# catniplab/vlgp

Hardware: AMD Instinct MI355X
Metric: EM iterations/sec (higher is better)
Workload: dtype f64

## Files before the change

### include/vlgp_hip.h

```cpp
#ifndef VLGP_HIP_H
#define VLGP_HIP_H

#include <stdint.h>

#ifdef __cplusplus
extern "C" {
#endif

#define VLGP_ABI_VERSION 3
#define VLGP_MAX_SETS 4
#define VLGP_MAX_L 64
#define VLGP_MAX_XDIM 64
#define VLGP_MAX_RANK 64
#define VLGP_UNIQUE_ID_BYTES 128

#define VLGP_OK 0
#define VLGP_ERR_ARG (-1)
#define VLGP_ERR_HIP (-2)
#define VLGP_ERR_STATE (-3)
#define VLGP_ERR_COMM (-4)

typedef struct vlgp_ctx vlgp_ctx;

int vlgp_abi_version(void);
// ... 138 lines not shown
#define VLGP_PATH_HSTEP_GENERIC 4
#define VLGP_PATH_HSTEP_OLD 5
#define VLGP_PATH_HSTEP_MIXED 6
int vlgp_debug_last_hstep_path(vlgp_ctx* ctx, int* path);
int vlgp_debug_reload_switches(vlgp_ctx* ctx);
int vlgp_debug_switch(vlgp_ctx* ctx, const char* name, double* value);
int vlgp_debug_live_memory(int64_t out[4]);
int vlgp_debug_hstep_stats(vlgp_ctx* ctx, double out[4]);
#define VLGP_HP_PATH 0
#define VLGP_HP_TC 1
#define VLGP_HP_N_LR 2
#define VLGP_HP_N_ROUGH 3
#define VLGP_HP_RMAX 4
#define VLGP_HP_CLASS 5
#define VLGP_HP_TABG 6
#define VLGP_HP_FUSED 7
#define VLGP_HP_NB 8
#define VLGP_HP_LDS 9
#define VLGP_HP_WLM 10
#define VLGP_HP_NW 11
#define VLGP_HP_TM_GLOBAL 12
#define VLGP_HP_HUGE 13
#define VLGP_HP_RERUN 14
#define VLGP_HP_RCAP 15
#define VLGP_HSTEP_PLAN_LEN 31
int vlgp_debug_hstep_plan(vlgp_ctx* ctx, int out[VLGP_HSTEP_PLAN_LEN]);
int vlgp_debug_mstep_plan(vlgp_ctx* ctx, int64_t rows, int out[12]);
#define VLGP_EP_FAMILY 0
#define VLGP_EP_DECLINE 1
#define VLGP_EP_LT 2
#define VLGP_EP_REC 3
#define VLGP_EP_MAXRA 4
#define VLGP_EP_USE_LANE 5
#define VLGP_EP_MIX 6
#define VLGP_EP_MAXRA_HI 7
#define VLGP_EP_RTOP 8
#define VLGP_EP_LO_SHG 9
#define VLGP_EP_N_LANES 10
#define VLGP_EP_CUT 11
#define VLGP_EP_CS 16
#define VLGP_EP_NJ 17
#define VLGP_EP_RP 18
#define VLGP_EP_RA 19
#define VLGP_EP_SMALL 20
#define VLGP_EP_RG 21
#define VLGP_EP_RANK 22
#define VLGP_EP_CLASS 38
#define VLGP_ESTEP_PLAN_LEN 54
// ... 24 lines not shown
```

### vlgp_amd/_lib.py

```python
import ctypes as C
import os

import numpy as np

os.environ.setdefault("HSA_ENABLE_IPC_MODE_LEGACY", "0")

_HERE = os.path.dirname(os.path.abspath(__file__))
LIB_PATH = os.path.join(_HERE, "libvlgp_hip.so")

ABI_VERSION = 3
MAX_SETS = 4
UNIQUE_ID_BYTES = 128
PROF_ESTEP, PROF_MSTEP, PROF_HSTEP, PROF_PRIOR = 0, 1, 2, 3
PROF_ESTEP_RA16, PROF_ESTEP_RA24, PROF_ESTEP_RA32, PROF_ESTEP_LONG, PROF_ESTEP_GENERIC = 4, 5, 6, 7, 8
PROF_ESTEP_PASS, PROF_ESTEP_FACTOR, PROF_ESTEP_MEAN = 9, 10, 11
PROF_HSTEP_LR, PROF_HSTEP_TAB = 12, 13
ESTEP_PATHS = ("none", "split", "fast", "long", "generic", "long_split", "split_mixed")
EP = dict(FAMILY=0, DECLINE=1, LT=2, REC=3, MAXRA=4, USE_LANE=5, MIX=6, MAXRA_HI=7, RTOP=8, LO_SHG=9, N_LANES=10, CUT=11, CS=16,
          NJ=17, RP=18, RA=19, SMALL=20, RG=21, RANK=22, CLASS=38)
ESTEP_PLAN_LEN = 54
ESPLIT = ("TAKEN", "OFF", "GENERIC", "L", "N", "LSPLIT_OFF", "LONG_RANK", "LONG_FEW", "SMALL_SET", "RANK", "REC")
ECLASS = ("LANE", "LO", "HI")
HP = dict(PATH=0, TC=1, N_LR=2, N_ROUGH=3, RMAX=4, CLASS=5, TABG=6, FUSED=7, NB=8, LDS=9, WLM=10, NW=11, TM_GLOBAL=12, HUGE=13,
          RERUN=14, RCAP=15)
HSTEP_PLAN_LEN = 31
HSTEP_PATHS = ("none", "lowrank", "dense", "big", "generic", "old", "mixed")
ERR_STATE = -3

_lib = None


class VlgpError(RuntimeError):

    status = detail = None


_dp = C.POINTER(C.c_double)
_ip = C.POINTER(C.c_int)
_i64p = C.POINTER(C.c_int64)
_u8p = C.POINTER(C.c_uint8)
_h = C.c_void_p

_SIGNATURES = {
    "vlgp_abi_version": (C.c_int, []),
    "vlgp_device_count": (C.c_int, [_ip]),
    "vlgp_create": (C.c_int, [C.c_int, C.c_int, C.c_int, C.c_int, C.c_int, _u8p, C.POINTER(_h)]),
    "vlgp_destroy": (C.c_int, [_h]),
    "vlgp_last_error": (C.c_char_p, [_h]),
# ... 149 lines not shown
```

### vlgp_amd/csrc/ctx.h

```cpp
#pragma once
#include <hip/hip_runtime.h>
#include <stdint.h>

#include <map>
#include <string>
#include <vector>

#include "../../include/vlgp_hip.h"
#include "dev_mem.h"

#define VLGP_WAVE 64
#define VLGP_E_LANES 4
#define VLGP_PRIOR_SLOTS 64

struct Prior {
    int T = 0;
    DevPtr<double> d_full;
    DevPtr<double> d_compact;
    std::vector<int> rl;
    std::vector<int64_t> goff;
    int64_t compact_len = 0;
    int index = -1;
};

// ... 62 lines not shown

#define VLGP_SWITCHES(X)                                                                                                 \
    X("VLGP_ESTEP_SPLIT", estep_split, TRI, -1, 0, 1, "split E-step (chip-wide launches per phase): 0 never, 1 whatever the set's size") \
    X("VLGP_ESTEP_LSPLIT", estep_lsplit, TRI, -1, 0, 1, "long units (T > 64) on the split E-step: 0 never, 1 below 128 tasks too") \
    X("VLGP_ESTEP_GENERIC", estep_generic, FLAG, false, 0, 1, "E-step: the generic kernels only (a replicated set keeps the split E-step)") \
    X("VLGP_ESTEP_LANEPT", estep_lanept, TRI, -1, 0, 1, "split E-step: 0 keeps the wave-per-task kernels for ranks <= 14") \
    X("VLGP_ESTEP_NO_SHARED_G", estep_no_shared_g, FLAG, false, 0, 1, "split E-step: per-wave staging of G in the rank <= 16 launches, no lane-per-task launches") \
    X("VLGP_ESTEP_MIX", estep_mix, TRI, -1, 0, 1, "split E-step: 0 launches lane-per-task and wave-per-task latents separately") \
    X("VLGP_ESTEP_LANES", estep_lanes, INT, 0, 1, VLGP_E_LANES, "split E-step: number of stream lanes (default: by set size, one or two)") \
    X("VLGP_LANE_PRIO", lane_prio, INT, 0, 0, 3, "instruction priority of the lane-per-task launches' waves")                \
    X("VLGP_LANE_CLOCK", lane_clock, INT, 0, 0, 2, "phase clock of the lane-per-task launches: 1 factor, 2 mean (vlgp_debug_phase_clock)") \
    X("VLGP_MSTEP_GENERIC", mstep_generic, FLAG, false, 0, 1, "M-step: the loop-based kernels at any size")                    \
    X("VLGP_MSTEP_WG_PER_CU", mstep_wg_per_cu, REAL, 1.0, 0.0, 1e300, "M-step accumulation: workgroups per compute unit")       \
    X("VLGP_NOISE_PASSES", noise_passes, FLAG, false, 0, 1, "M-step: the noise variance by two passes over the rows, not from the moments") \
    X("VLGP_NO_MGRAPH", no_mgraph, FLAG, false, 0, 1, "M-step: enqueue every launch instead of replaying the captured graph") \
    X("VLGP_ICHOL_BLOCK", ichol_block, FLAG, false, 0, 1, "prior factor: lengths <= 64 through the workgroup kernel of the long ones") \
    X("VLGP_NORMS_BLOCKS", norms_blocks, INT, 256, 1, 1024, "norms pass: largest number of workgroups (its partial sums have 1024 slots)") \
    X("VLGP_HSTEP_DENSE", hstep_dense, FLAG, false, 0, 1, "H-step: the dense matrix-pipe round, never the low-rank one")     \
    X("VLGP_HSTEP_GENERIC", hstep_generic, FLAG, false, 0, 1, "H-step: the generic kernels (the reference's omega retry)")     \
    X("VLGP_HSTEP_LOWRANK", hstep_lowrank, FLAG, false, 0, 1, "H-step: the low-rank round whatever the size rule says")        \
    X("VLGP_HSTEP_GENERIC_SEG", hstep_generic_seg, FLAG, false, 0, 1, "H-step: windows 65 ... 128 on the generic kernels")     \
    X("VLGP_HSTEP_FUSE_TABLES", hstep_fuse_tables, FLAG, false, 0, 1, "H-step: every low-rank round workgroup factors its kernel blocks itself (rejected: slower)") \
    X("VLGP_HSTEP_NO_WLM", hstep_no_wlm, FLAG, false, 0, 1, "H-step: the rounds read w row-major, no latent-major copy")       \
    X("VLGP_HSTEP_LR_TOL", hstep_lr_tol, REAL, 1e-12, 0.0, 1e300, "H-step: relative tolerance of the low-rank round's rank prediction") \
    X("VLGP_DEBUG_OCC", debug_occ, FLAG, false, 0, 1, "print occupancy of the fast E-step launch and the H-step's fall-backs on stderr")
#define VLGP_SW_T_FLAG bool
#define VLGP_SW_T_TRI int
#define VLGP_SW_T_INT int
#define VLGP_SW_T_REAL double
struct Switches {
#define X(name, field, kind, def, lo, hi, what) VLGP_SW_T_##kind field = def;
    VLGP_SWITCHES(X)
#undef X
};
void vlgp_read_switches(struct vlgp_ctx* ctx);

struct HostExchange;
enum { LANE_MAIN = 0, LANE_M = 1 };
struct CommLane {
    void* rccl = nullptr;
    HostExchange* shm = nullptr;
    hipStream_t stream = nullptr;
    bool open() const { return rccl || shm; }
};

struct ProfSlot {
// ... 37 lines not shown
    void* m_graph_exec = nullptr;
    std::vector<double> m_graph_key;

    DevPtr<double> d_ecols;
    DevPtr<int> d_fail;
    DevPtr<unsigned long long> d_clk;
    GrowBuf<double> d_work;
    HostGrowBuf<double> h_pinned;
    DevPtr<unsigned> d_hsync;
    HostPtr<double> h_hres;
    DevPtr<double> d_hres;
    unsigned h_seq = 0;
    GrowBuf<double> d_hmpart;
    bool hprep = false;
    DevEvent ev_e_done;
    bool e_done_valid = false;
    uint64_t hprep_epoch = 0, write_epoch = 0;
    GrowBuf<double> d_hmom;
    const UnitSet* hmom_us = nullptr;
    int hmom_T = 0;
    bool hmom_bracket = false;
    GrowBuf<double> d_hwlm;
    bool hwlm_valid = false;
    struct LrThr { int T; double dt, tol; std::vector<double> om; };
    std::vector<LrThr> lr_thr;
    Switches sw;
    std::vector<const void*> lds_attr_done;
    int h_prio = 1;
    double last_h_ms = 0.0, last_m_ms = 0.0;
    double h_t0 = 0.0;
    int last_hstep_path = 0;
    double hstat[4] = {0.0, 0.0, 0.0, 0.0};
    int hplan[VLGP_HSTEP_PLAN_LEN] = {};

    bool prof_on = false;
    ProfSlot prof[VLGP_PROF_KINDS];
    struct PendingProf { int kind; DevEvent a, b; double units; bool done; };
    std::vector<PendingProf> pending;

    CommLane lanes[2];
    HostExchange* hx = nullptr;
    int rank = 0, world = 1;

    DevStream elane[VLGP_E_LANES - 1];
    DevEvent ev_e_fork, ev_e_join[VLGP_E_LANES - 1];
    int last_estep_path = 0;
// ... 175 lines not shown
```

### vlgp_amd/csrc/hstep.hip

```cpp
#include <stdio.h>
#include <stdlib.h>
#include <string.h>

#include <algorithm>

#include "ctx.h"
#include "wave_tri.h"
#include "hstep_mfma.h"
#include "hstep_lr.h"

#define HS_MAXT 1024

struct HPrepArgs {
    int T;
    double dt;
    const double* logp;
    double* kinv;
    double* q;
    double* dk;
    double* scal;
    double* tm;
    double* km;
};

// ... 564 lines not shown
    mom[(int64_t)l * TT + idx] = a;
}

struct HRoundArgs {
    HFastArgs F;
    int n_eval, nb;
    int lds_doubles;
    unsigned seq;
    unsigned* sync;
    const double* mom;
    double* qsum;
    double* red;
    double* host;
    HLrTabArgs lr;
    unsigned total_blocks;
    int k_blocks;
    int lr_nev;
    int lr_ev[16];
    int slot_stride;
    int nbe[16];
    unsigned lr_mask;
    unsigned long long* clk;
    int prio;
};

template <int T, int NW, bool ONESET>
struct HRoundK {
    using G = HmGeom<T>;
    static constexpr int LDK = T | 2;
    static constexpr int TASKW = ONESET ? HmGeom50::TASK : G::TASK;
    static constexpr int SHR = ONESET ? HmGeom50::SHARED : 0;
    static constexpr int KBLK = TASKW + T * LDK + SHR;
};

template <int T, int NW, bool ONESET>
__device__ __forceinline__ void hstep_round_kblock(const HRoundArgs& R, int e, double* lds, double* kvs, double (*part)[2],
                                                   int lane, int wid) {
    using G = HmGeom<T>;
    using KG = HRoundK<T, NW, ONESET>;
    constexpr int LDK = KG::LDK, TASKW = KG::TASKW;
    const HFastArgs& A = R.F;
    double* buf = lds;
    double* Kl = lds + TASKW;
    double* dks = kvs + HmGeom50::KVN;
    double preC[(T + 3) / 4];
    constexpr bool PRE = NW >= (T + 15) / 16;
// ... 193 lines not shown
            if (!ok) { tr = nan(""); cs = nan(""); }
            for (int o = 32; o > 0; o >>= 1) {
                tr += __shfl_xor(tr, o, 64);
                cs += __shfl_xor(cs, o, 64);
            }
            tr -= (double)(T - A.Tr);
        }
        if (lane == 0) {
            part[wid][0] = tr;
            part[wid][1] = cs;
        }
    }
    hstep_round_finish<NW>(R, lds, part, &s_last, out_slot);
}

__global__ void __launch_bounds__(128) hstep_lr_tables(HRoundArgs R) {
    __shared__ double kv[64], dkv[64];
    __shared__ int s_i[4];
    hstep_wave_prio(R.prio);
    const int e = R.lr_ev[blockIdx.x];
    lr_tables_block<128>(R.lr, e, exp(R.F.logp[3 * e + 0]), exp(R.F.logp[3 * e + 1]), kv, dkv, s_i);
}

#ifndef HLR64_LB
#define HLR64_LB 4
#endif
template <int T, int NW, int RC, bool TABG = false, bool TABF = false>
__global__ void __launch_bounds__(64 * NW, RC <= 24 ? (T == 64 ? HLR64_LB : 4) : 3) hstep_round_lr(HRoundArgs R) {
    hstep_wave_prio(R.prio);
    constexpr bool ONESET = T == 50;
    constexpr int NK = T == 50 ? 7 : 8;
    using KG = HRoundK<T, NW, ONESET>;
    extern __shared__ __attribute__((aligned(16))) double lds_dyn[];
    __shared__ double part[NW][2];
    __shared__ int s_last;
    const HFastArgs& A = R.F;
    const int lane = threadIdx.x & 63, wid = threadIdx.x >> 6;
    int64_t out_slot = -1;
    if ((int)blockIdx.x < R.k_blocks) {
        hstep_round_kblock<T, NW, ONESET>(R, blockIdx.x, lds_dyn, lds_dyn + KG::KBLK - KG::SHR, part, lane, wid);
    } else {
        const int b = blockIdx.x - R.k_blocks;
        const int ei = b / R.nb, bx = b - ei * R.nb;
        const int e = R.lr_ev[ei];
        out_slot = (int64_t)e * R.slot_stride + bx;
        double tr = 0.0, cs = 0.0;
        const double eps = exp(A.logp[3 * e + 2]);
        if constexpr (TABF)
            lr_group<RC, NK, NW, false, true>(nullptr, LrMeta{}, nullptr,
                             A.wlm ? A.wlm + (int64_t)A.latent[e] * A.wld : A.w, A.off, A.wlm ? 1 : A.L,
                             A.wlm ? 0 : A.latent[e], A.M, A.Tr, eps, 16 * bx, lds_dyn, lane, wid, tr, cs,
                             b == 0 ? R.clk : nullptr, &R.lr, e, exp(A.logp[3 * e + 0]), exp(A.logp[3 * e + 1]),
                             R.lds_doubles, bx == 0);
        else
        lr_group<RC, NK, NW, TABG>(R.lr.tab + (int64_t)e * 2 * LR_TROWS * LR_RCAP, R.lr.meta[e], R.lr.pairs + (int64_t)e * LR_NPAIR,
                             A.wlm ? A.wlm + (int64_t)A.latent[e] * A.wld : A.w, A.off, A.wlm ? 1 : A.L,
                             A.wlm ? 0 : A.latent[e], A.M, A.Tr, eps, 16 * bx, lds_dyn, lane, wid, tr, cs,
                             b == 0 ? R.clk : nullptr);
        if (lane == 0) {
            part[wid][0] = wid == 0 ? tr : 0.0;
            part[wid][1] = wid == 0 ? cs : 0.0;
        }
    }
    hstep_round_finish<NW>(R, lds_dyn, part, &s_last, out_slot);
}

static int lr_host_rank(int T, double dt, double omega, double tol) {
    const int h = T / 2, nt = (T + 1) / 2;
    const bool odd = (T & 1) != 0;
    std::vector<double> kv(T);
    for (int d = 0; d < T; ++d) kv[d] = exp(-omega * (d * dt) * (d * dt));
    const double RS2 = 0.70710678118654752440;
    int total = 0;
    for (int par = 0; par < 2; ++par) {
        const int n = par == 0 ? nt : h;
        auto kent = [&](int t, int p) {
            const int d1 = t > p ? t - p : p - t, d2 = T - 1 - t - p;
            if (par == 0) {
                const double s = ((odd && t == h) ? RS2 : 1.0) * ((odd && p == h) ? RS2 : 1.0);
                return s * (kv[d1] + kv[d2]);
            }
// ... 57 lines not shown
}

static int launch_hstep_impl(vlgp_ctx* ctx, UnitSet& us, int window, double dt, int n_eval, const int* latent,
                             const double* logp, double* ll, double* dll, bool force_dense);

int launch_hstep(vlgp_ctx* ctx, UnitSet& us, int window, double dt, int n_eval, const int* latent,
                 const double* logp, double* ll, double* dll) {
    return launch_hstep_impl(ctx, us, window, dt, n_eval, latent, logp, ll, dll, false);
}

static bool hstep_round_kernels_apply(vlgp_ctx* ctx, const UnitSet& us, int T) {
    const Switches& sw = ctx->sw;
    return us.Tmin == T && us.Tmax == T && T <= 64 && T >= (sw.hstep_dense ? 24 : 4) && !sw.hstep_generic;
}
static int hstep_prepare_units(vlgp_ctx* ctx, UnitSet& us, int T, bool want_wlm, bool want_mom, hipStream_t st) {
    const int L = ctx->L, M = us.M;
    if (want_wlm && (!ctx->hwlm_valid || ctx->hmom_us != &us)) {
        const int64_t n = us.rows * L;
        HIPCHK(ctx, ctx->d_hwlm.ensure(n, n));
        hipLaunchKernelGGL(hstep_w_latent_major, dim3((unsigned)((n + 255) / 256)), dim3(256), 0, st, L,
                           us.rows, us.w, ctx->d_hwlm);
        HIPCHK(ctx, hipGetLastError());
        ctx->hwlm_valid = true;
    }
    if (!want_mom) return VLGP_OK;
    const int HT = T <= 50 ? 50 : 64;
    constexpr int NCH = 64;
    const int64_t n_mom = (int64_t)L * HT * HT;
    if (ctx->d_hmom.len < n_mom || ctx->d_hmpart.len < n_mom * NCH) {
        ctx->hmom_us = nullptr;
        HIPCHK(ctx, ctx->d_hmom.ensure(n_mom, n_mom));
        HIPCHK(ctx, ctx->d_hmpart.ensure(n_mom * NCH, n_mom * NCH));
    }
    if (ctx->hmom_us != &us || ctx->hmom_T != T) {
        if (HT == 50)
            hipLaunchKernelGGL((hstep_moment_kernel<50>), dim3(NCH, L), dim3(256), 0, st, L, M, T,
                               us.d_off, us.mu, NCH, ctx->d_hmpart);
        else
            hipLaunchKernelGGL((hstep_moment_kernel<64>), dim3(NCH, L), dim3(256), 0, st, L, M, T,
                               us.d_off, us.mu, NCH, ctx->d_hmpart);
        hipLaunchKernelGGL(hstep_moment_reduce, dim3((HT * HT + 255) / 256, L), dim3(256), 0, st, NCH,
                           HT * HT, ctx->d_hmpart, ctx->d_hmom);
        HIPCHK(ctx, hipGetLastError());
        ctx->hmom_us = &us;
        ctx->hmom_T = T;
    }
    return VLGP_OK;
}
int hstep_prepare(vlgp_ctx* ctx, UnitSet& us, int T, hipStream_t st) {
    if (!hstep_round_kernels_apply(ctx, us, T)) return VLGP_OK;
    ctx->hmom_us = nullptr;
    ctx->hwlm_valid = false;
    return hstep_prepare_units(ctx, us, T, !ctx->sw.hstep_no_wlm, true, st);
}

static int launch_hstep_impl(vlgp_ctx* ctx, UnitSet& us, int window, double dt, int n_eval, const int* latent,
                             const double* logp, double* ll, double* dll, bool force_dense) {
    const int T = window, L = ctx->L, M = us.M;
    if (T > HS_MAXT) return vlgp_fail(ctx, VLGP_ERR_ARG, "H-step kernel supports window <= %d, got %d", HS_MAXT, T);
    const bool huge = (size_t)(T * (T | 1)) * 8 > 150 * 1024;
    if (us.Tmin != T || us.Tmax != T)
        return vlgp_fail(ctx, VLGP_ERR_STATE, "H-step needs every unit to have exactly window=%d rows", T);
    const Switches& sw = ctx->sw;
    const bool lr_allowed = !force_dense && !sw.hstep_dense;
    const bool fast = T <= 64 && T >= (lr_allowed ? 4 : 24) && !sw.hstep_generic;
    const int TC = T <= 50 ? 50 : 64;
    const int64_t TT = fast ? (int64_t)TC * TC : (int64_t)T * T;
    const int64_t o_kinv = 0, o_q = o_kinv + n_eval * TT, o_dk = o_q + n_eval * TT, o_scal = o_dk + n_eval * TT;
    const int64_t o_out = o_scal + 4 * n_eval, o_red = o_out + 2LL * n_eval * M, o_logp = o_red + 3 * n_eval;
    const int64_t o_lat = o_logp + 3 * n_eval, o_qsum = o_lat + n_eval + 8, o_mpart = o_qsum + 2 * n_eval + 2;
    const int64_t o_tm = o_mpart;
    const int64_t o_km = o_tm + (T > 64 ? n_eval * TT : 0);
    const int64_t o_bmat = o_km + (huge ? (int64_t)n_eval * T * (T | 1) : 0);
    const int64_t o_lrtab = (o_bmat + (huge ? (int64_t)n_eval * M * T * (T | 1) : 0) + 1) & ~1LL;
    const int64_t o_lrmeta = o_lrtab + (fast ? (int64_t)n_eval * 2 * LR_TROWS * LR_RCAP : 0);
    const int64_t o_lrpairs = o_lrmeta + (fast ? (int64_t)n_eval * 4 : 0);
// ... 62 lines not shown
                const double gens = (double)n_lr * m_rule / 4000.0;
                const double extra = gens > 1.0 ? gens - 1.0 : 0.0;
                const double t_dense = 41.0 + 28.0 * extra, t_lr = 13.0 + base[ci] + marg[ci] * extra;
                if (T >= 24 && t_lr > 0.95 * t_dense) lr = false;
            }
            const bool mixed = lr && n_rough > 0;
            const int nb_lr = (M + 15) / 16, nb_dense = (M + MFMA_NW - 1) / MFMA_NW;
            R.n_eval = n_eval; R.nb = lr ? nb_lr : nb_dense;
            R.slot_stride = mixed ? nb_dense : R.nb;
            R.lr_mask = 0;
            for (int e = 0; e < n_eval; ++e) {
                const bool e_lr = lr && !((rough >> e) & 1u);
                R.nbe[e] = e_lr ? nb_lr : nb_dense;
                if (e_lr) R.lr_mask |= 1u << e;
                R.lr_ev[e] = e;
            }
            R.seq = ++ctx->h_seq; R.sync = ctx->d_hsync;
            R.mom = ctx->d_hmom; R.qsum = W + o_qsum;
            R.red = W + o_red;
            R.lr.tab = nullptr; R.lr.meta = nullptr; R.lr.pairs = nullptr;
            R.total_blocks = (unsigned)(n_eval + n_lr_or_all(lr, n_lr, n_eval) * (lr ? nb_lr : nb_dense) + (mixed ? n_rough * nb_dense : 0));
            R.k_blocks = n_eval; R.lr_nev = n_eval; R.clk = ctx->d_clk;
            R.prio = ctx->h_prio;
            if (lr) {
                R.lr.T = T; R.lr.dt = dt; R.lr.tol = lr_tol;
                for (int e = 0; e < n_eval; ++e) R.lr.rcap[e] = rcap[e];
                R.lr.tab = W + o_lrtab;
                R.lr.meta = reinterpret_cast<LrMeta*>(W + o_lrmeta);
                R.lr.pairs = reinterpret_cast<unsigned short*>(W + o_lrpairs);
                const bool fuse_tables = sw.hstep_fuse_tables && rmax <= 24;
                if (!fuse_tables) {
                    HRoundArgs Rt = R;
                    int k = 0;
                    for (int e = 0; e < n_eval; ++e)
                        if ((R.lr_mask >> e) & 1u) Rt.lr_ev[k++] = e;
                    vlgp_prof_begin(ctx, VLGP_PROF_HSTEP_TAB);
                    hipLaunchKernelGGL(hstep_lr_tables, dim3(n_lr), dim3(128), 0, ctx->stream, Rt);
                    vlgp_prof_end(ctx, VLGP_PROF_HSTEP_TAB, (double)n_lr);
                }
                HIPCHK(ctx, hipGetLastError());
                ctx->hstat[0] += n_lr;
                for (int e = 0; e < n_eval; ++e) ctx->hstat[1] += rcap[e];
                ctx->hstat[2] += n_rough;
            } else if (mfma) {
                ctx->hstat[2] += n_eval;
            }
// ... 221 lines not shown
```

### vlgp_amd/csrc/hstep_lr.h

```cpp
#pragma once
#include <hip/hip_runtime.h>
#include <stdint.h>

#include "hstep_mfma.h"

#define LR_RCAP 32
#define LR_RH 20
#define LR_TROWS 32
#define LR_NPAIR 576

struct LrMeta {
    int re, ro;
    int r;
    int ns_tiles;
    int n_tiles;
    int overflow;
    int pad0, pad1;
};

struct HLrTabArgs {
    int T;
    double dt, tol;
    int rcap[16];
    double* tab;
// ... 183 lines not shown
        if (j <= i) {
            const bool io = i >= re, jo = j >= re;
            int pos;
            if (io == jo)
                pos = io ? n_ee + (i - re) * (i - re + 1) / 2 + (j - re) : i * (i + 1) / 2 + j;
            else
                pos = ns16 + (i - re) * re + j;
            pairs[pos] = (unsigned short)((i << 8) | j);
        }
    }
    if (threadIdx.x == 0) {
        LrMeta m;
        m.re = re;
        m.ro = ro;
        m.r = rt;
        m.ns_tiles = ns16 >> 4;
        m.n_tiles = (ns16 + nc16) >> 4;
        m.overflow = overflow;
        m.pad0 = m.pad1 = 0;
        A.meta[e] = m;
    }
}

struct LrGeom {
    int LDU, NPS;
    int o_u, o_ud, o_mp, o_xb, o_red, o_codes, total;
};
__host__ __device__ constexpr bool lr_block_inverse(int rc) {
#ifdef LR_ROWWISE
    return false;
#else
    return rc <= 28;
#endif
}
__host__ __device__ constexpr int lr_xs_per_wave(int rc) {
    if (!lr_block_inverse(rc)) return 64;
    const int gb = rc <= 16 ? 4 : 5, bs = (rc + gb - 1) / gb, lps = gb * (gb + 1) / 2, spw = 64 / lps;
    return (spw * gb * bs + 1) & ~1;
}
__host__ __device__ inline LrGeom lr_geom(int r, int ntp, int nw, bool tab_global, int rc) {
    LrGeom G;
    G.LDU = tab_global ? LR_RCAP : ((r + 1) | 1);
    G.NPS = (r * (r + 1) / 2 + 2) | 1;
    G.o_u = 0;
    G.o_ud = tab_global ? 0 : ntp * G.LDU;
    G.o_mp = tab_global ? 0 : ((2 * ntp * G.LDU + 1) & ~1);
    G.o_xb = (G.o_mp + 16 * G.NPS + 1) & ~1;
    G.o_red = G.o_xb;
    const int xw = nw * lr_xs_per_wave(rc), rw = nw * 32 + 2;
    G.o_codes = G.o_xb + (xw > rw ? xw : rw);
    int ncode = r * (r + 1) / 2 + 32;
    if (ncode > LR_NPAIR) ncode = LR_NPAIR;
    G.total = G.o_codes + (ncode + 3) / 4;
    return G;
}

template <int RC, int NK, int NW, bool TABG = false, bool TABF = false>
__device__ __forceinline__ void lr_group(const double* __restrict__ tab_e, const LrMeta mt,
                                         const unsigned short* __restrict__ pairs_e, const double* __restrict__ w,
                                         const int64_t* __restrict__ off, int L, int l, int M, int T, double eps,
                                         int seg0, double* lds, int lane, int wid, double& out_tr, double& out_cs,
                                         unsigned long long* clk = nullptr, const HLrTabArgs* fa = nullptr, int e = 0,
                                         double sigmasq = 0.0, double omega = 0.0, int lds_doubles = 0, bool publish = false) {
    static_assert(!(TABG && TABF), "fused tables live in LDS");
    long long tck = clk ? clock64() : 0;
    auto stamp = [&](int slot) {
        if (clk && threadIdx.x == 0) {
            const long long now = clock64();
            atomicAdd(clk + slot, (unsigned long long)(now - tck));
            tck = now;
        }
    };
    const int c = lane & 15, g = lane >> 4;
    const int h = T >> 1, nt = (T + 1) >> 1;
    const int gs = seg0 + c;
    const bool sval = gs < M;
    const int64_t r0 = sval ? (int64_t)gs * T : 0;
    (void)off;
    double wpre1[NK], wpre2[NK];
    auto load_w = [&]() {
#pragma unroll
        for (int kk = 0; kk < NK; ++kk) {
            const int tau = 4 * kk + g;
            wpre1[kk] = (sval && tau < nt) ? w[(r0 + tau) * L + l] : 0.0;
            wpre2[kk] = (sval && tau < h) ? w[(r0 + T - 1 - tau) * L + l] : 0.0;
        }
    };
    if constexpr (!TABF) load_w();
    constexpr int TPRE = (TABG || TABF) ? 1 : (4 * NK * LR_RCAP + 64 * NW - 1) / (64 * NW);
    double tpre[TPRE][2];
    LrMeta mloc = mt;
    constexpr int FR = TABF ? LR_RH : 1;
    double fg[FR], fgd[FR];
    int f_r = 0, f_cap = 0, f_tau = 0, f_re = 0;
    bool f_rowin = false;
    if constexpr (TABF) {
        double* kv = lds + lds_doubles - 136;
        double* dkv = kv + 64;
        int* s_i = reinterpret_cast<int*>(dkv + 64);
        if (threadIdx.x < 64) {
            const double d = lane * fa->dt, d2 = d * d;
            const double k = lane < T ? exp(-omega * d2) : 0.0;
            kv[lane] = k;
            dkv[lane] = -omega * d2 * k;
        }
        __syncthreads();
        lr_factor_wave(T, fa->tol, wid, lane, kv, dkv, fg, fgd, f_r, f_cap, f_rowin, f_tau);
        if (lane == 0 && wid < 2) {
            s_i[wid] = f_r;
            s_i[2 + wid] = f_cap;
        }
// ... 68 lines not shown
                else
                    pos = ns16 + (i - re) * re + j;
                codes[pos] = (unsigned short)((i << 8) | j);
            }
        }
    }
    if constexpr (!TABG && !TABF) {
        double* Uw = lds + G.o_u;
        double* Udw = lds + G.o_ud;
#pragma unroll
        for (int q = 0; q < TPRE; ++q) {
            const int x = threadIdx.x + q * 64 * NW;
            const int tau = x >> 5, cc = x & 31;
            if (x < 4 * NK * LR_RCAP && cc < LDU) {
                Uw[tau * LDU + cc] = tpre[q][0];
                Udw[tau * LDU + cc] = tpre[q][1];
            }
        }
        if (LDU > LR_RCAP && threadIdx.x < 4 * NK) {
            Uw[threadIdx.x * LDU + LR_RCAP] = 0.0;
            Udw[threadIdx.x * LDU + LR_RCAP] = 0.0;
        }
    }
    double ap[NK], am[NK], bp[NK], bm[NK];
    double dsum = 0.0;
    auto weights = [&](const double* p1, const double* p2) {
        dsum = 0.0;
#pragma unroll
        for (int kk = 0; kk < NK; ++kk) {
            const int tau = 4 * kk + g;
            const bool in1 = sval && tau < nt, in2 = sval && tau < h;
            const double w1 = p1 ? p1[kk] : (in1 ? w[(r0 + tau) * L + l] : 0.0);
            const double w2 = p2 ? p2[kk] : (in2 ? w[(r0 + T - 1 - tau) * L + l] : 0.0);
            const double d1 = lr_rcp(fma(eps, w1, 1.0)), d2 = lr_rcp(fma(eps, w2, 1.0));
            const double t1 = w1 * d1, t2 = w2 * d2;
            const double q1 = t1 * d1, q2 = t2 * d2;
            const double fa = in2 ? 0.5 : 1.0;
            ap[kk] = fa * (t1 + t2);
            bp[kk] = fa * (q1 + q2);
            am[kk] = in2 ? 0.5 * (t1 - t2) : 0.0;
            bm[kk] = in2 ? 0.5 * (q1 - q2) : 0.0;
            dsum += (in1 ? d1 : 0.0) + (in2 ? d2 : 0.0);
        }
    };
    weights(wpre1, wpre2);
    __syncthreads();
    stamp(0);
    auto tile_codes = [&](int q, int& i, int& j, int& idx, double& dg) {
        const unsigned code = codes[q * 16 + c];
        const bool valid = code != 0xffffu;
        i = valid ? (int)(code >> 8) : r;
        j = valid ? (int)(code & 255u) : r;
        idx = valid ? i * (i + 1) / 2 + j : NPZ;
        dg = (valid && i == j) ? 1.0 : 0.0;
    };
    auto phase1 = [&](int qb, int qe, const double(&aw)[NK]) {
        for (int q = qb + wid; q < qe; q += 2 * NW) {
            const bool two = q + NW < qe;
            int i0, j0, x0, i1, j1, x1;
            double g0, g1;
            tile_codes(q, i0, j0, x0, g0);
            tile_codes(two ? q + NW : q, i1, j1, x1, g1);
            const double* u0i = Ul + g * LDU + i0;
            const double* u0j = Ul + g * LDU + j0;
            const double* u1i = Ul + g * LDU + i1;
            const double* u1j = Ul + g * LDU + j1;
            hm_d4 acc0 = hm_d4{0.0, 0.0, 0.0, 0.0}, acc1 = hm_d4{0.0, 0.0, 0.0, 0.0};
            if (two) {
// ... 145 lines not shown
                    tri_wave_order();
                }
            };
            sweeps();
            const int base = rowv * (rowv + 1) / 2;
#pragma unroll
            for (int j = 0; j < RC; ++j)
                if (j < r) Ms[(rowok && j <= rowv) ? base + j : NPZ + 1] = j == rowv ? -a[j] : -2.0 * a[j];
        }
    }
    }
    __syncthreads();
    stamp(2);
    double ts[4] = {0.0, 0.0, 0.0, 0.0}, cs[4] = {0.0, 0.0, 0.0, 0.0};
    double wa[NK], wb[NK];
    auto weights_kind = [&](int kind) {
        double ds = 0.0;
#pragma unroll
        for (int kk = 0; kk < NK; ++kk) {
            const int tau = 4 * kk + g;
            const bool in1 = sval && tau < nt, in2 = sval && tau < h;
            const double w1 = in1 ? w[(r0 + tau) * L + l] : 0.0;
            const double w2 = in2 ? w[(r0 + T - 1 - tau) * L + l] : 0.0;
            const double d1 = lr_rcp(fma(eps, w1, 1.0)), d2 = lr_rcp(fma(eps, w2, 1.0));
            const double t1 = w1 * d1, t2 = w2 * d2;
            const double q1 = t1 * d1, q2 = t2 * d2;
            const double fa = in2 ? 0.5 : 1.0;
            if (kind == 0) {
                wa[kk] = fa * (t1 + t2);
                wb[kk] = fa * (q1 + q2);
                ds += (in1 ? d1 : 0.0) + (in2 ? d2 : 0.0);
            } else {
                wa[kk] = in2 ? 0.5 * (t1 - t2) : 0.0;
                wb[kk] = in2 ? 0.5 * (q1 - q2) : 0.0;
            }
        }
        if (kind == 0) dsum = ds;
    };
    auto tile3 = [&](int q) {
        const unsigned code = codes[q * 16 + c];
        const bool valid = code != 0xffffu;
        const int i = valid ? (int)(code >> 8) : r, j = valid ? (int)(code & 255u) : r;
        const double* ui = Ul + g * LDU + i;
        const double* uj = Ul + g * LDU + j;
        const double* di = Udl + g * LDU + i;
        const double* dj = Udl + g * LDU + j;
        hm_d4 accB = hm_d4{0.0, 0.0, 0.0, 0.0}, accD = hm_d4{0.0, 0.0, 0.0, 0.0};
#pragma unroll
        for (int kk = 0; kk < NK; ++kk) {
            const int o = 4 * kk * LDU;
            const double vi = ui[o], vj = uj[o];
            const double pb = vi * vj;
            const double pd = fma(di[o], vj, vi * dj[o]);
            accB = __builtin_amdgcn_mfma_f64_16x16x4f64(wb[kk], pb, accB, 0, 0, 0);
            accD = __builtin_amdgcn_mfma_f64_16x16x4f64(wa[kk], pd, accD, 0, 0, 0);
        }
        const int idx = valid ? i * (i + 1) / 2 + j : NPZ;
#pragma unroll
        for (int p = 0; p < 4; ++p) {
            const double m = Mp[(g + 4 * p) * NPS + idx];
            ts[p] = fma(m, accB[p], ts[p]);
            cs[p] = fma(m, accD[p], cs[p]);
        }
    };
    weights_kind(0);
    dsum += __shfl_xor(dsum, 16, 64);
    dsum += __shfl_xor(dsum, 32, 64);
    for (int q = wid; q < ns_tiles; q += NW) tile3(q);
    weights_kind(1);
    for (int q = ns_tiles + ((wid - ns_tiles % NW) + NW) % NW; q < n_tiles; q += NW) tile3(q);
#pragma unroll
    for (int p = 0; p < 4; ++p) {
        const double tsum = lr_row_sum_to15(ts[p]), csum = lr_row_sum_to15(cs[p]);
        if (c == 15) {
            red[(wid * 16 + g + 4 * p) * 2 + 0] = tsum;
            red[(wid * 16 + g + 4 * p) * 2 + 1] = csum;
        }
    }
    __syncthreads();
    if (wid == 0) {
        double t = 0.0, cc = 0.0;
#pragma unroll
        for (int wv = 0; wv < NW; ++wv) {
            t += red[(wv * 16 + c) * 2 + 0];
            cc += red[(wv * 16 + c) * 2 + 1];
        }
        double tA = (sval && g == 0) ? dsum - t : 0.0;
        double cv = (sval && g == 0) ? cc : 0.0;
#pragma unroll
        for (int o = 1; o < 16; o <<= 1) {
            tA += __shfl_xor(tA, o, 64);
            cv += __shfl_xor(cv, o, 64);
// ... 7 lines not shown
```

### vlgp_amd/engine.py

```python
import collections
import ctypes as C
import logging
import os
import time

import numpy as np

from . import _lib
from ._lib import VlgpError, check, dptr, i64ptr, iptr, u8ptr

logger = logging.getLogger(__name__)

__all__ = ["Engine", "DeviceTrials", "estep", "mstep", "hstep", "update_w", "update_v",
           "make_cholesky", "infer", "vem", "constrain_loading", "constrain_latent", "VlgpError"]


TRACE = {}


def _f64(a):
    return np.ascontiguousarray(a, dtype=np.float64)


def _all_ones(x):
# ... 619 lines not shown
        p = C.c_int(0)
        self._ck(self.lib.vlgp_debug_last_estep_path(self.h, C.byref(p)))
        return _lib.ESTEP_PATHS[p.value]

    @property
    def last_hstep_path(self):
        p = C.c_int(0)
        self._ck(self.lib.vlgp_debug_last_hstep_path(self.h, C.byref(p)))
        return _lib.HSTEP_PATHS[p.value]

    def reload_switches(self):
        self._ck(self.lib.vlgp_debug_reload_switches(self.h))

    def switch(self, name):
        v = C.c_double(0)
        self._ck(self.lib.vlgp_debug_switch(self.h, name.encode(), C.byref(v)))
        return v.value

    def hstep_stats(self):
        out = np.zeros(4)
        self._ck(self.lib.vlgp_debug_hstep_stats(self.h, dptr(out)))
        return out

    def hstep_plan(self):
        out = np.zeros(_lib.HSTEP_PLAN_LEN, dtype=np.int32)
        self._ck(self.lib.vlgp_debug_hstep_plan(self.h, iptr(out)))
        o = [int(v) for v in out]
        at = lambda name: o[_lib.HP[name]]
        return dict(path=_lib.HSTEP_PATHS[at("PATH")], rerun=at("RERUN"), TC=at("TC"), nb=at("NB"), wlm=at("WLM"),
                    n_lr=at("N_LR"), n_rough=at("N_ROUGH"), rmax=at("RMAX"), rc=at("CLASS"), tabg=at("TABG"), fused=at("FUSED"),
                    lds=at("LDS"), rcap=o[_lib.HP["RCAP"]:_lib.HP["RCAP"] + 16], nw=at("NW"), tm_global=at("TM_GLOBAL"),
                    huge=at("HUGE"))

    MSTEP_PLAN_KEYS = ("G", "rows_per_wg", "CT", "S", "nthr", "tiles", "LT", "PT", "exact", "fixed", "anyg", "noise_passes")

    def mstep_plan(self, rows):
        out = np.zeros(12, dtype=np.int32)
        self._ck(self.lib.vlgp_debug_mstep_plan(self.h, C.c_int64(int(rows)), iptr(out)))
        return dict(zip(self.MSTEP_PLAN_KEYS, (int(v) for v in out)))

    ESTEP_MODES = {"estep": 1 | 2 | 4, "update_w": 4, "update_v": 1 | 8}
    ESPLIT_DECLINES = ("taken", "VLGP_ESTEP_SPLIT=0", "VLGP_ESTEP_GENERIC", "L > 10", "N > 1024", "VLGP_ESTEP_LSPLIT=0",
                       "long rank", "long: few tasks", "small set", "rank > 32", "records")
    ECLASSES = tuple(k.lower() for k in _lib.ECLASS)

    def estep_plan(self, set_id, n_iter, what="estep", vb=True):
        mode = self.ESTEP_MODES[what] | (8 if what == "estep" and vb else 0)
        out = np.zeros(_lib.ESTEP_PLAN_LEN, dtype=np.int32)
        self._ck(self.lib.vlgp_debug_estep_plan(self.h, int(set_id), mode, int(n_iter), iptr(out)))
        o = [int(v) for v in out]
        at = lambda name: o[_lib.EP[name]]
        per_latent = lambda name: o[_lib.EP[name]:_lib.EP[name] + min(self.L, 16)]
        family = _lib.ESTEP_PATHS[at("FAMILY")]
        plan = {"family": family, "decline": self.ESPLIT_DECLINES[at("DECLINE")]}
        if family in ("split", "split_mixed", "long_split"):
# ... 460 lines not shown
```

Baseline: 154.4.

## Cache folded H-step low-rank weights in a per-latent device table

Adds a device table that holds the folded weights (ap, am, the two weight kinds and the d-sum) for each latent and 16-row segment. A separate build kernel fills it whenever the latent-major w copy or that latent's log-eps changes. The low-rank round kernels then read those weights instead of recomputing reciprocals and folds from w on every evaluation. This trades recurring ALU work and w loads for extra memory, an extra build launch, and host-side bookkeeping of generation and eps bits, with a size cap set by a new switch.

```diff
diff --git a/include/vlgp_hip.h b/include/vlgp_hip.h
--- a/include/vlgp_hip.h
+++ b/include/vlgp_hip.h
@@ -184,8 +184,9 @@
 #define VLGP_HP_TM_GLOBAL 12
 #define VLGP_HP_HUGE 13
 #define VLGP_HP_RERUN 14
-#define VLGP_HP_RCAP 15
-#define VLGP_HSTEP_PLAN_LEN 31
+#define VLGP_HP_WTAB 15
+#define VLGP_HP_RCAP 16
+#define VLGP_HSTEP_PLAN_LEN 32
 int vlgp_debug_hstep_plan(vlgp_ctx* ctx, int out[VLGP_HSTEP_PLAN_LEN]);
 int vlgp_debug_mstep_plan(vlgp_ctx* ctx, int64_t rows, int out[12]);
 #define VLGP_EP_FAMILY 0
diff --git a/vlgp_amd/_lib.py b/vlgp_amd/_lib.py
--- a/vlgp_amd/_lib.py
+++ b/vlgp_amd/_lib.py
@@ -22,8 +22,8 @@
 ESPLIT = ("TAKEN", "OFF", "GENERIC", "L", "N", "LSPLIT_OFF", "LONG_RANK", "LONG_FEW", "SMALL_SET", "RANK", "REC")
 ECLASS = ("LANE", "LO", "HI")
 HP = dict(PATH=0, TC=1, N_LR=2, N_ROUGH=3, RMAX=4, CLASS=5, TABG=6, FUSED=7, NB=8, LDS=9, WLM=10, NW=11, TM_GLOBAL=12, HUGE=13,
-          RERUN=14, RCAP=15)
-HSTEP_PLAN_LEN = 31
+          RERUN=14, WTAB=15, RCAP=16)
+HSTEP_PLAN_LEN = 32
 HSTEP_PATHS = ("none", "lowrank", "dense", "big", "generic", "old", "mixed")
 ERR_STATE = -3
 
diff --git a/vlgp_amd/csrc/ctx.h b/vlgp_amd/csrc/ctx.h
--- a/vlgp_amd/csrc/ctx.h
+++ b/vlgp_amd/csrc/ctx.h
@@ -108,6 +108,7 @@
     X("VLGP_HSTEP_GENERIC_SEG", hstep_generic_seg, FLAG, false, 0, 1, "H-step: windows 65 ... 128 on the generic kernels")     \
     X("VLGP_HSTEP_FUSE_TABLES", hstep_fuse_tables, FLAG, false, 0, 1, "H-step: every low-rank round workgroup factors its kernel blocks itself (rejected: slower)") \
     X("VLGP_HSTEP_NO_WLM", hstep_no_wlm, FLAG, false, 0, 1, "H-step: the rounds read w row-major, no latent-major copy")       \
+    X("VLGP_HSTEP_WTAB", hstep_wtab, INT, 256, 0, 65536, "H-step: largest folded-weights table of a bracket's low-rank rounds in MiB (0: the rounds compute their weights)") \
     X("VLGP_HSTEP_LR_TOL", hstep_lr_tol, REAL, 1e-12, 0.0, 1e300, "H-step: relative tolerance of the low-rank round's rank prediction") \
     X("VLGP_DEBUG_OCC", debug_occ, FLAG, false, 0, 1, "print occupancy of the fast E-step launch and the H-step's fall-backs on stderr")
 #define VLGP_SW_T_FLAG bool
@@ -191,6 +192,13 @@
     bool hmom_bracket = false;
     GrowBuf<double> d_hwlm;
     bool hwlm_valid = false;
+    GrowBuf<double> d_hwtab;
+    uint64_t hwlm_gen = 0;
+    int hwtab_T = 0;
+    unsigned long long hwtab_known = 0;
+    std::vector<double> hwtab_logeps;
+    std::vector<uint64_t> hwtab_gen;
+    std::vector<uint64_t> hwtab_seen;
     struct LrThr { int T; double dt, tol; std::vector<double> om; };
     std::vector<LrThr> lr_thr;
     Switches sw;
diff --git a/vlgp_amd/csrc/hstep.hip b/vlgp_amd/csrc/hstep.hip
--- a/vlgp_amd/csrc/hstep.hip
+++ b/vlgp_amd/csrc/hstep.hip
@@ -610,6 +610,8 @@
     unsigned lr_mask;
     unsigned long long* clk;
     int prio;
+    const double* wtab;
+    unsigned wtab_mask;
 };
 
 template <int T, int NW, bool ONESET>
@@ -849,6 +851,22 @@
     lr_tables_block<128>(R.lr, e, exp(R.F.logp[3 * e + 0]), exp(R.F.logp[3 * e + 1]), kv, dkv, s_i);
 }
 
+struct HWtabArgs {
+    int M, T, nb;
+    const double* wlm;
+    int64_t wld;
+    double* tab;
+    unsigned long long mask;
+    double logeps[VLGP_MAX_L];
+};
+template <int NK>
+__global__ void __launch_bounds__(256) hstep_lr_wtab(HWtabArgs A) {
+    const int l = blockIdx.y, grp = blockIdx.x * 4 + (threadIdx.x >> 6);
+    if (!((A.mask >> l) & 1ull) || grp >= A.nb) return;
+    lr_wtab_build<NK>(A.wlm + (int64_t)l * A.wld, 1, 0, A.M, A.T, exp(A.logeps[l]), 16 * grp, threadIdx.x & 63,
+                      A.tab + ((int64_t)l * A.nb + grp) * lr_wtab_block(NK));
+}
+
 #ifndef HLR64_LB
 #define HLR64_LB 4
 #endif
@@ -873,6 +891,7 @@
         out_slot = (int64_t)e * R.slot_stride + bx;
         double tr = 0.0, cs = 0.0;
         const double eps = exp(A.logp[3 * e + 2]);
+        const double* wt = ((R.wtab_mask >> e) & 1u) ? R.wtab + ((int64_t)A.latent[e] * R.nb + bx) * lr_wtab_block(NK) : nullptr;
         if constexpr (TABF)
             lr_group<RC, NK, NW, false, true>(nullptr, LrMeta{}, nullptr,
                              A.wlm ? A.wlm + (int64_t)A.latent[e] * A.wld : A.w, A.off, A.wlm ? 1 : A.L,
@@ -883,7 +902,7 @@
         lr_group<RC, NK, NW, TABG>(R.lr.tab + (int64_t)e * 2 * LR_TROWS * LR_RCAP, R.lr.meta[e], R.lr.pairs + (int64_t)e * LR_NPAIR,
                              A.wlm ? A.wlm + (int64_t)A.latent[e] * A.wld : A.w, A.off, A.wlm ? 1 : A.L,
                              A.wlm ? 0 : A.latent[e], A.M, A.Tr, eps, 16 * bx, lds_dyn, lane, wid, tr, cs,
-                             b == 0 ? R.clk : nullptr);
+                             b == 0 ? R.clk : nullptr, nullptr, 0, 0.0, 0.0, 0, false, wt);
         if (lane == 0) {
             part[wid][0] = wid == 0 ? tr : 0.0;
             part[wid][1] = wid == 0 ? cs : 0.0;
@@ -987,6 +1006,7 @@
                            us.rows, us.w, ctx->d_hwlm);
         HIPCHK(ctx, hipGetLastError());
         ctx->hwlm_valid = true;
+        ++ctx->hwlm_gen;
     }
     if (!want_mom) return VLGP_OK;
     const int HT = T <= 50 ? 50 : 64;
@@ -1012,11 +1032,44 @@
     }
     return VLGP_OK;
 }
+static bool hstep_wtab_applies(vlgp_ctx* ctx, const UnitSet& us, int T) {
+    const Switches& sw = ctx->sw;
+    if (sw.hstep_wtab <= 0 || sw.hstep_no_wlm || sw.hstep_dense || sw.hstep_fuse_tables || T > 64 || ctx->L > 64) return false;
+    const int64_t n = (int64_t)ctx->L * ((us.M + 15) / 16) * lr_wtab_block(T <= 50 ? 7 : 8);
+    return n * 8 <= (int64_t)sw.hstep_wtab << 20;
+}
+static int hstep_wtab_build(vlgp_ctx* ctx, UnitSet& us, int T, unsigned long long mask, hipStream_t st) {
+    const int L = ctx->L, nb = (us.M + 15) / 16, NK = T <= 50 ? 7 : 8;
+    const int64_t n = (int64_t)L * nb * lr_wtab_block(NK);
+    if (ctx->d_hwtab.len < n) {
+        HIPCHK(ctx, ctx->d_hwtab.ensure(n, n));
+        ctx->hwtab_gen.assign(L, 0);
+    }
+    ctx->hwtab_gen.resize(L, 0);
+    HWtabArgs A;
+    A.M = us.M; A.T = T; A.nb = nb; A.wlm = ctx->d_hwlm; A.wld = us.rows; A.tab = ctx->d_hwtab; A.mask = mask;
+    for (int l = 0; l < L; ++l) A.logeps[l] = ctx->hwtab_logeps[l];
+    const dim3 grid((unsigned)((nb + 3) / 4), (unsigned)L);
+    if (NK == 7) hipLaunchKernelGGL(hstep_lr_wtab<7>, grid, dim3(256), 0, st, A);
+    else hipLaunchKernelGGL(hstep_lr_wtab<8>, grid, dim3(256), 0, st, A);
+    HIPCHK(ctx, hipGetLastError());
+    for (int l = 0; l < L; ++l)
+        if ((mask >> l) & 1ull) ctx->hwtab_gen[l] = ctx->hwlm_gen;
+    ctx->hwtab_T = T;
+    return VLGP_OK;
+}
+static bool same_bits(double a, double b) { return memcmp(&a, &b, sizeof(double)) == 0; }
+
 int hstep_prepare(vlgp_ctx* ctx, UnitSet& us, int T, hipStream_t st) {
     if (!hstep_round_kernels_apply(ctx, us, T)) return VLGP_OK;
     ctx->hmom_us = nullptr;
     ctx->hwlm_valid = false;
-    return hstep_prepare_units(ctx, us, T, !ctx->sw.hstep_no_wlm, true, st);
+    CHK(hstep_prepare_units(ctx, us, T, !ctx->sw.hstep_no_wlm, true, st));
+    if (hstep_wtab_applies(ctx, us, T) && ctx->hwlm_valid && ctx->hwtab_known) {
+        ctx->hwtab_logeps.resize(ctx->L, 0.0);
+        CHK(hstep_wtab_build(ctx, us, T, ctx->hwtab_known, st));
+    }
+    return VLGP_OK;
 }
 
 static int launch_hstep_impl(vlgp_ctx* ctx, UnitSet& us, int window, double dt, int n_eval, const int* latent,
@@ -1125,6 +1178,33 @@
             R.total_blocks = (unsigned)(n_eval + n_lr_or_all(lr, n_lr, n_eval) * (lr ? nb_lr : nb_dense) + (mixed ? n_rough * nb_dense : 0));
             R.k_blocks = n_eval; R.lr_nev = n_eval; R.clk = ctx->d_clk;
             R.prio = ctx->h_prio;
+            R.wtab = nullptr; R.wtab_mask = 0;
+            if (lr && F.wlm && hstep_wtab_applies(ctx, us, T)) {
+                ctx->hwtab_logeps.resize(L, 0.0);
+                ctx->hwtab_gen.resize(L, 0);
+                ctx->hwtab_seen.resize(L, 0);
+                if (ctx->hwtab_T != T) ctx->hwtab_gen.assign(L, 0);
+                unsigned long long rebuild = 0;
+                for (int e = 0; e < n_eval; ++e) {
+                    if ((rough >> e) & 1u) continue;
+                    const int l = latent[e];
+                    const double le = logp[3 * e + 2];
+                    const bool built = ctx->hwtab_gen[l] == ctx->hwlm_gen && ((ctx->hwtab_known >> l) & 1ull);
+                    if (built && same_bits(ctx->hwtab_logeps[l], le)) {
+                        R.wtab_mask |= 1u << e;
+                    } else if (ctx->hwtab_seen[l] != ctx->hwlm_gen) {
+                        ctx->hwtab_logeps[l] = le;
+                        ctx->hwtab_known |= 1ull << l;
+                        ctx->hwtab_gen[l] = ctx->hwlm_gen;
+                        rebuild |= 1ull << l;
+                        R.wtab_mask |= 1u << e;
+                    }
+                    ctx->hwtab_seen[l] = ctx->hwlm_gen;
+                }
+                if (rebuild) CHK(hstep_wtab_build(ctx, us, T, rebuild, ctx->stream));
+                R.wtab = ctx->d_hwtab;
+            }
+            hplan[VLGP_HP_WTAB] = (int)R.wtab_mask;
             if (lr) {
                 R.lr.T = T; R.lr.dt = dt; R.lr.tol = lr_tol;
                 for (int e = 0; e < n_eval; ++e) R.lr.rcap[e] = rcap[e];
diff --git a/vlgp_amd/csrc/hstep_lr.h b/vlgp_amd/csrc/hstep_lr.h
--- a/vlgp_amd/csrc/hstep_lr.h
+++ b/vlgp_amd/csrc/hstep_lr.h
@@ -229,6 +229,79 @@
     }
 }
 
+struct LrFoldRow {
+    double d1, d2, t1, t2;
+    double fa;
+    bool in1, in2;
+};
+__device__ __forceinline__ LrFoldRow lr_fold_row(double w1, double w2, double eps, bool in1, bool in2) {
+#pragma clang fp contract(off)
+    LrFoldRow f;
+    f.d1 = lr_rcp(fma(eps, w1, 1.0));
+    f.d2 = lr_rcp(fma(eps, w2, 1.0));
+    f.t1 = w1 * f.d1;
+    f.t2 = w2 * f.d2;
+    f.fa = in2 ? 0.5 : 1.0;
+    f.in1 = in1;
+    f.in2 = in2;
+    return f;
+}
+__device__ __forceinline__ void lr_fold_phase1(const LrFoldRow& f, double& ap, double& am) {
+#pragma clang fp contract(off)
+    ap = f.fa * (f.t1 + f.t2);
+    am = f.in2 ? 0.5 * (f.t1 - f.t2) : 0.0;
+}
+__device__ __forceinline__ void lr_fold_phase3(const LrFoldRow& f, double w1, int kind, double& wa, double& wb) {
+#pragma clang fp contract(off)
+    const double q2 = f.d2 * f.t2;
+    if (kind == 0) {
+        wa = f.fa * fma(w1, f.d1, f.t2);
+        wb = f.fa * fma(f.d1, f.t1, q2);
+    } else {
+        wa = f.in2 ? 0.5 * fma(w1, f.d1, -f.t2) : 0.0;
+        wb = f.in2 ? 0.5 * fma(f.d1, f.t1, -q2) : 0.0;
+    }
+}
+__device__ __forceinline__ double lr_fold_dsum(const LrFoldRow& f) { return (f.in1 ? f.d1 : 0.0) + (f.in2 ? f.d2 : 0.0); }
+
+#define LR_WT_AP 0
+#define LR_WT_AM 1
+#define LR_WT_K0 2
+__host__ __device__ constexpr int lr_wtab_block(int nk) { return (6 * nk + 1) * 64; }
+
+template <int NK>
+__device__ __forceinline__ void lr_wtab_build(const double* __restrict__ w, int L, int l, int M, int T, double eps, int seg0,
+                                              int lane, double* __restrict__ out) {
+    const int c = lane & 15, g = lane >> 4;
+    const int h = T >> 1, nt = (T + 1) >> 1;
+    const int gs = seg0 + c;
+    const bool sval = gs < M;
+    const int64_t r0 = sval ? (int64_t)gs * T : 0;
+    double dsum = 0.0;
+#pragma unroll
+    for (int kk = 0; kk < NK; ++kk) {
+        const int tau = 4 * kk + g;
+        const bool in1 = sval && tau < nt, in2 = sval && tau < h;
+        const double w1 = in1 ? w[(r0 + tau) * L + l] : 0.0;
+        const double w2 = in2 ? w[(r0 + T - 1 - tau) * L + l] : 0.0;
+        const LrFoldRow f = lr_fold_row(w1, w2, eps, in1, in2);
+        double ap, am, wa0, wb0, wa1, wb1;
+        lr_fold_phase1(f, ap, am);
+        lr_fold_phase3(f, w1, 0, wa0, wb0);
+        lr_fold_phase3(f, w1, 1, wa1, wb1);
+        out[(LR_WT_AP * NK + kk) * 64 + lane] = ap;
+        out[(LR_WT_AM * NK + kk) * 64 + lane] = am;
+        out[((LR_WT_K0 + 0) * NK + kk) * 64 + lane] = wa0;
+        out[((LR_WT_K0 + 1) * NK + kk) * 64 + lane] = wb0;
+        out[((LR_WT_K0 + 2) * NK + kk) * 64 + lane] = wa1;
+        out[((LR_WT_K0 + 3) * NK + kk) * 64 + lane] = wb1;
+        dsum += lr_fold_dsum(f);
+    }
+    dsum += __shfl_xor(dsum, 16, 64);
+    dsum += __shfl_xor(dsum, 32, 64);
+    if (g == 0) out[6 * NK * 64 + c] = dsum;
+}
+
 struct LrGeom {
     int LDU, NPS;
     int o_u, o_ud, o_mp, o_xb, o_red, o_codes, total;
@@ -268,8 +341,10 @@
                                          const int64_t* __restrict__ off, int L, int l, int M, int T, double eps,
                                          int seg0, double* lds, int lane, int wid, double& out_tr, double& out_cs,
                                          unsigned long long* clk = nullptr, const HLrTabArgs* fa = nullptr, int e = 0,
-                                         double sigmasq = 0.0, double omega = 0.0, int lds_doubles = 0, bool publish = false) {
+                                         double sigmasq = 0.0, double omega = 0.0, int lds_doubles = 0, bool publish = false,
+                                         const double* __restrict__ wt = nullptr) {
     static_assert(!(TABG && TABF), "fused tables live in LDS");
+    const bool wtab = !TABF && wt != nullptr;
     long long tck = clk ? clock64() : 0;
     auto stamp = [&](int slot) {
         if (clk && threadIdx.x == 0) {
@@ -293,7 +368,18 @@
             wpre2[kk] = (sval && tau < h) ? w[(r0 + T - 1 - tau) * L + l] : 0.0;
         }
     };
-    if constexpr (!TABF) load_w();
+    double ap[NK], am[NK];
+    if constexpr (!TABF) {
+        if (wtab) {
+#pragma unroll
+            for (int kk = 0; kk < NK; ++kk) {
+                ap[kk] = wt[(LR_WT_AP * NK + kk) * 64 + lane];
+                am[kk] = wt[(LR_WT_AM * NK + kk) * 64 + lane];
+            }
+        } else {
+            load_w();
+        }
+    }
     constexpr int TPRE = (TABG || TABF) ? 1 : (4 * NK * LR_RCAP + 64 * NW - 1) / (64 * NW);
     double tpre[TPRE][2];
     LrMeta mloc = mt;
@@ -408,28 +494,18 @@
             Udw[threadIdx.x * LDU + LR_RCAP] = 0.0;
         }
     }
-    double ap[NK], am[NK], bp[NK], bm[NK];
     double dsum = 0.0;
     auto weights = [&](const double* p1, const double* p2) {
-        dsum = 0.0;
 #pragma unroll
         for (int kk = 0; kk < NK; ++kk) {
             const int tau = 4 * kk + g;
             const bool in1 = sval && tau < nt, in2 = sval && tau < h;
             const double w1 = p1 ? p1[kk] : (in1 ? w[(r0 + tau) * L + l] : 0.0);
             const double w2 = p2 ? p2[kk] : (in2 ? w[(r0 + T - 1 - tau) * L + l] : 0.0);
-            const double d1 = lr_rcp(fma(eps, w1, 1.0)), d2 = lr_rcp(fma(eps, w2, 1.0));
-            const double t1 = w1 * d1, t2 = w2 * d2;
-            const double q1 = t1 * d1, q2 = t2 * d2;
-            const double fa = in2 ? 0.5 : 1.0;
-            ap[kk] = fa * (t1 + t2);
-            bp[kk] = fa * (q1 + q2);
-            am[kk] = in2 ? 0.5 * (t1 - t2) : 0.0;
-            bm[kk] = in2 ? 0.5 * (q1 - q2) : 0.0;
-            dsum += (in1 ? d1 : 0.0) + (in2 ? d2 : 0.0);
-        }
-    };
-    weights(wpre1, wpre2);
+            lr_fold_phase1(lr_fold_row(w1, w2, eps, in1, in2), ap[kk], am[kk]);
+        }
+    };
+    if (!wtab) weights(wpre1, wpre2);
     __syncthreads();
     stamp(0);
     auto tile_codes = [&](int q, int& i, int& j, int& idx, double& dg) {
@@ -621,20 +697,23 @@
             const bool in1 = sval && tau < nt, in2 = sval && tau < h;
             const double w1 = in1 ? w[(r0 + tau) * L + l] : 0.0;
             const double w2 = in2 ? w[(r0 + T - 1 - tau) * L + l] : 0.0;
-            const double d1 = lr_rcp(fma(eps, w1, 1.0)), d2 = lr_rcp(fma(eps, w2, 1.0));
-            const double t1 = w1 * d1, t2 = w2 * d2;
-            const double q1 = t1 * d1, q2 = t2 * d2;
-            const double fa = in2 ? 0.5 : 1.0;
-            if (kind == 0) {
-                wa[kk] = fa * (t1 + t2);
-                wb[kk] = fa * (q1 + q2);
-                ds += (in1 ? d1 : 0.0) + (in2 ? d2 : 0.0);
-            } else {
-                wa[kk] = in2 ? 0.5 * (t1 - t2) : 0.0;
-                wb[kk] = in2 ? 0.5 * (q1 - q2) : 0.0;
-            }
-        }
-        if (kind == 0) dsum = ds;
+            const LrFoldRow f = lr_fold_row(w1, w2, eps, in1, in2);
+            lr_fold_phase3(f, w1, kind, wa[kk], wb[kk]);
+            if (kind == 0) ds += lr_fold_dsum(f);
+        }
+        if (kind == 0) {
+            ds += __shfl_xor(ds, 16, 64);
+            ds += __shfl_xor(ds, 32, 64);
+            dsum = ds;
+        }
+    };
+    auto table_kind = [&](int kind) {
+#pragma unroll
+        for (int kk = 0; kk < NK; ++kk) {
+            wa[kk] = wt[((LR_WT_K0 + 2 * kind) * NK + kk) * 64 + lane];
+            wb[kk] = wt[((LR_WT_K0 + 2 * kind + 1) * NK + kk) * 64 + lane];
+        }
+        if (kind == 0) dsum = wt[6 * NK * 64 + c];
     };
     auto tile3 = [&](int q) {
         const unsigned code = codes[q * 16 + c];
@@ -662,11 +741,11 @@
             cs[p] = fma(m, accD[p], cs[p]);
         }
     };
-    weights_kind(0);
-    dsum += __shfl_xor(dsum, 16, 64);
-    dsum += __shfl_xor(dsum, 32, 64);
+    if (wtab) table_kind(0);
+    else weights_kind(0);
     for (int q = wid; q < ns_tiles; q += NW) tile3(q);
-    weights_kind(1);
+    if (wtab) table_kind(1);
+    else weights_kind(1);
     for (int q = ns_tiles + ((wid - ns_tiles % NW) + NW) % NW; q < n_tiles; q += NW) tile3(q);
 #pragma unroll
     for (int p = 0; p < 4; ++p) {
diff --git a/vlgp_amd/engine.py b/vlgp_amd/engine.py
--- a/vlgp_amd/engine.py
+++ b/vlgp_amd/engine.py
@@ -665,15 +665,18 @@
         self._ck(self.lib.vlgp_debug_hstep_stats(self.h, dptr(out)))
         return out
 
-    def hstep_plan(self):
+    def hstep_plan(self, weights=False):
         out = np.zeros(_lib.HSTEP_PLAN_LEN, dtype=np.int32)
         self._ck(self.lib.vlgp_debug_hstep_plan(self.h, iptr(out)))
         o = [int(v) for v in out]
         at = lambda name: o[_lib.HP[name]]
-        return dict(path=_lib.HSTEP_PATHS[at("PATH")], rerun=at("RERUN"), TC=at("TC"), nb=at("NB"), wlm=at("WLM"),
+        plan = dict(path=_lib.HSTEP_PATHS[at("PATH")], rerun=at("RERUN"), TC=at("TC"), nb=at("NB"), wlm=at("WLM"),
                     n_lr=at("N_LR"), n_rough=at("N_ROUGH"), rmax=at("RMAX"), rc=at("CLASS"), tabg=at("TABG"), fused=at("FUSED"),
                     lds=at("LDS"), rcap=o[_lib.HP["RCAP"]:_lib.HP["RCAP"] + 16], nw=at("NW"), tm_global=at("TM_GLOBAL"),
                     huge=at("HUGE"))
+        if weights:
+            plan["wtab"] = [(at("WTAB") >> e) & 1 for e in range(16)]
+        return plan
 
     MSTEP_PLAN_KEYS = ("G", "rows_per_wg", "CT", "S", "nthr", "tiles", "LT", "PT", "exact", "fixed", "anyg", "noise_passes")
 
```

After: 154.7 (median of 2 runs). Within noise of the previous version (+0.2%).
